# zhizdev/sparsefusion

Hardware: AMD Instinct MI355X
Metric: novel views/sec, distillation steps (2 NGP renders fwd+bwd + VAE enc/dec + 51-eval PLMS + LPIPS), 256^2 / 32x32 latents, 2-view synthetic hydrant (higher is better)
Workload: dtype bf16 MFMA operands / f32 accumulate (UNet); f32 (NGP render)

## Files before the change

### sparsefusion_amd/csrc/ngp_bwd_mfma.h

```cpp
#pragma once
#include "sf_dev.h"
#include "ngp_device.h"

#define FB_PTS 32
#define FB_SF 33
#define FB_SH 65
#define FB_WAVE_FLOATS (FB_PTS * FB_SF + 2 * FB_PTS * FB_SH + FB_PTS * 4 + FB_PTS)
#define FB_W0 0
#define FB_W1 (FB_W0 + NGP_HID * FB_SF)
#define FB_W2 (FB_W1 + NGP_HID * FB_SH)
#define FB_B0 (FB_W2 + NGP_OUT * NGP_HID)
#define FB_B1 (FB_B0 + NGP_HID)
#define FB_B2 (FB_B1 + NGP_HID)
#define FB_WTOT (FB_B2 + 8)
#define FB_LDS_FLOATS (FB_WTOT + 4 * FB_WAVE_FLOATS)

struct FBArgs {
  const float* table; const float* w0; const float* b0; const float* w1; const float* b1; const float* w2; const float* b2;
  float bound;
  long long* g_w0; long long* g_b0; long long* g_w1; long long* g_b1; long long* g_w2; long long* g_b2;
  float* f_w0; float* f_b0; float* f_w1; float* f_b1; float* f_w2; float* f_b2;
  float thr;
  NgpLevels lv;
  const float* rays_o; const float* rays_d; const float* aabb; const float* z_s; const float* dsig; const float* drgb;
  float* dfeat_out;
  uint32_t P, T2;
  uint32_t dfeat_P, p_off;
  const float* feat_c; const float* feat_f; const uint32_t* perm;
};

SF_KERNEL(256) void k_ngp_field_bwd_mfma(FBArgs a) {
  SF_DYN_LDS(lds_raw);
  float* W = reinterpret_cast<float*>(lds_raw);
  const int tid = threadIdx.x, lane = tid & 63, wave = tid >> 6;
  float* F = W + FB_WTOT + wave * FB_WAVE_FLOATS;
  float* H1 = F + FB_PTS * FB_SF;
  float* H2 = H1 + FB_PTS * FB_SH;
  float* DO = H2 + FB_PTS * FB_SH;
  float* INS = DO + FB_PTS * 4;
  for (int i = tid; i < NGP_HID * NGP_FEAT; i += 256) W[FB_W0 + (i >> 5) * FB_SF + (i & 31)] = a.w0[i];
  for (int i = tid; i < NGP_HID * NGP_HID; i += 256) W[FB_W1 + (i >> 6) * FB_SH + (i & 63)] = a.w1[i];
  for (int i = tid; i < NGP_OUT * NGP_HID; i += 256) W[FB_W2 + i] = a.w2[i];
  if (tid < NGP_HID) { W[FB_B0 + tid] = a.b0[tid]; W[FB_B1 + tid] = a.b1[tid]; }
  if (tid < NGP_OUT) W[FB_B2 + tid] = a.b2[tid];
  float box[6];
#pragma unroll
  for (int i = 0; i < 6; ++i) box[i] = a.aabb[i];
  sf_sync();

  const int li = lane & 15, kq = lane >> 4;
  f32x4 acc1[4][4], acc0[4][2];
#pragma unroll
  for (int i = 0; i < 4; ++i) {
#pragma unroll
    for (int j = 0; j < 4; ++j) acc1[i][j] = f32x4{0.f, 0.f, 0.f, 0.f};
    acc0[i][0] = f32x4{0.f, 0.f, 0.f, 0.f};
    acc0[i][1] = f32x4{0.f, 0.f, 0.f, 0.f};
  }
  float acc2[4] = {0.f, 0.f, 0.f, 0.f};
  float accb2 = 0.0f, accb1 = 0.0f, accb0 = 0.0f;

  const uint32_t n_trips = (a.P + FB_PTS - 1) / FB_PTS;
  for (uint32_t trip = blockIdx.x * 4 + wave; trip < n_trips; trip += gridDim.x * 4) {
    const uint32_t p0 = trip * FB_PTS;
    const int pl = lane & 31, half = lane >> 5;
    const uint32_t p = p0 + pl;
    const bool live = p < a.P;
    float x[3] = {0.f, 0.f, 0.f}, x01[3] = {0.f, 0.f, 0.f};
    bool inside = false;
    if (live) {
      const uint32_t n = p / a.T2;
      const float o[3] = {a.rays_o[n * 3], a.rays_o[n * 3 + 1], a.rays_o[n * 3 + 2]};
      const float d[3] = {a.rays_d[n * 3], a.rays_d[n * 3 + 1], a.rays_d[n * 3 + 2]};
      ngp_point(o, d, a.z_s[p], box, x);
      inside = ngp_unit(x, a.bound, x01);
    }
    if (a.feat_c) {
      f32x4 fv[4];
#pragma unroll
      for (int j = 0; j < 4; ++j) fv[j] = f32x4{0.f, 0.f, 0.f, 0.f};
      if (live) {
        const uint32_t pg = a.p_off + p, n = pg / a.T2, T = a.T2 >> 1;
        const uint32_t src = a.perm[pg];
        const float* row = (src < T ? a.feat_c + ((size_t)n * T + src) * NGP_FEAT : a.feat_f + ((size_t)n * T + (src - T)) * NGP_FEAT) + half * 16;
#pragma unroll
        for (int j = 0; j < 4; ++j) fv[j] = *reinterpret_cast<const f32x4*>(row + 4 * j);
      }
#pragma unroll
      for (int j = 0; j < 4; ++j)
#pragma unroll
        for (int e = 0; e < 4; ++e) F[pl * FB_SF + half * 16 + 4 * j + e] = fv[j][e];
    } else {
#pragma unroll
      for (int ll = 0; ll < 8; ++ll) {
        const uint32_t l = half * 8 + ll;
        float r0 = 0.0f, r1 = 0.0f;
        if (inside && l < a.lv.L) {
          NgpCell c;
          ngp_cell(a.lv, l, x01, c);
          const float* tab = a.table + (size_t)a.lv.offset[l] * 2;
#pragma unroll
          for (int i = 0; i < 8; ++i) {
            const f32x2 fv = *reinterpret_cast<const f32x2*>(tab + (size_t)c.row[i] * 2);
            r0 = fmaf(c.w[i], fv[0], r0);
            r1 = fmaf(c.w[i], fv[1], r1);
          }
        }
        F[pl * FB_SF + 2 * l] = r0;
        F[pl * FB_SF + 2 * l + 1] = r1;
      }
    }
    if (half == 0) INS[pl] = inside ? 1.0f : 0.0f;
    sf_wave_sync();

    {
      f32x4 c[2][4];
#pragma unroll
      for (int nt = 0; nt < 4; ++nt) {
        const float bv = W[FB_B0 + nt * 16 + li];
        c[0][nt] = f32x4{bv, bv, bv, bv};
        c[1][nt] = c[0][nt];
      }
#pragma unroll
      for (int s = 0; s < NGP_FEAT / 4; ++s) {
        const float a0 = F[li * FB_SF + 4 * s + kq], a1 = F[(16 + li) * FB_SF + 4 * s + kq];
#pragma unroll
        for (int nt = 0; nt < 4; ++nt) {
          const float b = W[FB_W0 + (nt * 16 + li) * FB_SF + 4 * s + kq];
          c[0][nt] = sf_mfma4(a0, b, c[0][nt]);
          c[1][nt] = sf_mfma4(a1, b, c[1][nt]);
        }
      }
#pragma unroll
      for (int mt = 0; mt < 2; ++mt)
#pragma unroll
        for (int nt = 0; nt < 4; ++nt)
#pragma unroll
          for (int r = 0; r < 4; ++r) H1[(mt * 16 + 4 * kq + r) * FB_SH + nt * 16 + li] = fmaxf(c[mt][nt][r], 0.0f);
    }
    sf_wave_sync();
    {
      f32x4 c[2][4];
#pragma unroll
      for (int nt = 0; nt < 4; ++nt) {
        const float bv = W[FB_B1 + nt * 16 + li];
        c[0][nt] = f32x4{bv, bv, bv, bv};
        c[1][nt] = c[0][nt];
      }
#pragma unroll
      for (int s = 0; s < NGP_HID / 4; ++s) {
        const float a0 = H1[li * FB_SH + 4 * s + kq], a1 = H1[(16 + li) * FB_SH + 4 * s + kq];
#pragma unroll
        for (int nt = 0; nt < 4; ++nt) {
          const float b = W[FB_W1 + (nt * 16 + li) * FB_SH + 4 * s + kq];
          c[0][nt] = sf_mfma4(a0, b, c[0][nt]);
          c[1][nt] = sf_mfma4(a1, b, c[1][nt]);
        }
      }
#pragma unroll
      for (int mt = 0; mt < 2; ++mt)
#pragma unroll
        for (int nt = 0; nt < 4; ++nt)
#pragma unroll
          for (int r = 0; r < 4; ++r) H2[(mt * 16 + 4 * kq + r) * FB_SH + nt * 16 + li] = fmaxf(c[mt][nt][r], 0.0f);
    }
    sf_wave_sync();
    {
      float o0 = W[FB_B2 + 2 * half], o1 = W[FB_B2 + 2 * half + 1];
#pragma unroll 8
      for (int k = 0; k < NGP_HID; ++k) {
        const float hk = H2[pl * FB_SH + k];
        o0 = fmaf(W[FB_W2 + (2 * half) * NGP_HID + k], hk, o0);
        o1 = fmaf(W[FB_W2 + (2 * half + 1) * NGP_HID + k], hk, o1);
      }
      float d0 = 0.0f, d1 = 0.0f;
      if (live) {
        if (half == 0) {
          const float pre = o0 + ngp_blob(x);
          d0 = a.dsig[p] * expf(fminf(fmaxf(pre, -15.0f), 15.0f));
          const float sg = ngp_sigmoid(o1);
          d1 = a.drgb[p * 3 + 0] * sg * (1.0f - sg);
        } else {
          const float s0 = ngp_sigmoid(o0), s1 = ngp_sigmoid(o1);
          d0 = a.drgb[p * 3 + 1] * s0 * (1.0f - s0);
          d1 = a.drgb[p * 3 + 2] * s1 * (1.0f - s1);
        }
      }
      DO[pl * 4 + 2 * half] = d0;
      DO[pl * 4 + 2 * half + 1] = d1;
    }
    sf_wave_sync();
    {
      float b = 0.0f;
#pragma unroll 4
      for (int q = 0; q < FB_PTS; ++q) {
        const float dv = DO[q * 4 + kq];
#pragma unroll
        for (int i = 0; i < 4; ++i) acc2[i] = fmaf(dv, H2[q * FB_SH + 4 * li + i], acc2[i]);
        b += dv;
      }
      if (li == 0) accb2 += b;
    }
    sf_wave_sync();
    {
      const float w0 = W[FB_W2 + lane], w1 = W[FB_W2 + NGP_HID + lane], w2 = W[FB_W2 + 2 * NGP_HID + lane],
                  w3 = W[FB_W2 + 3 * NGP_HID + lane];
      float b = 0.0f;
#pragma unroll 4
      for (int q = 0; q < FB_PTS; ++q) {
        const f32x4 dv = *reinterpret_cast<const f32x4*>(DO + q * 4);
        const float g = fmaf(w3, dv[3], fmaf(w2, dv[2], fmaf(w1, dv[1], w0 * dv[0])));
        const float m = H2[q * FB_SH + lane] > 0.0f ? g : 0.0f;
        H2[q * FB_SH + lane] = m;
        b += m;
      }
      accb1 += b;
    }
    sf_wave_sync();
#pragma unroll
    for (int s = 0; s < FB_PTS / 4; ++s) {
      float av[4], bv[4];
#pragma unroll
      for (int t = 0; t < 4; ++t) {
        av[t] = H2[(4 * s + kq) * FB_SH + t * 16 + li];
        bv[t] = H1[(4 * s + kq) * FB_SH + t * 16 + li];
      }
#pragma unroll
      for (int jt = 0; jt < 4; ++jt)
#pragma unroll
        for (int kt = 0; kt < 4; ++kt) acc1[jt][kt] = sf_mfma4(av[jt], bv[kt], acc1[jt][kt]);
    }
    {
      f32x4 c[2][4];
#pragma unroll
      for (int nt = 0; nt < 4; ++nt) { c[0][nt] = f32x4{0.f, 0.f, 0.f, 0.f}; c[1][nt] = c[0][nt]; }
#pragma unroll
      for (int s = 0; s < NGP_HID / 4; ++s) {
        const float a0 = H2[li * FB_SH + 4 * s + kq], a1 = H2[(16 + li) * FB_SH + 4 * s + kq];
#pragma unroll
        for (int nt = 0; nt < 4; ++nt) {
          const float b = W[FB_W1 + (4 * s + kq) * FB_SH + nt * 16 + li];
          c[0][nt] = sf_mfma4(a0, b, c[0][nt]);
          c[1][nt] = sf_mfma4(a1, b, c[1][nt]);
        }
      }
      sf_wave_sync();
#pragma unroll
      for (int mt = 0; mt < 2; ++mt)
#pragma unroll
        for (int nt = 0; nt < 4; ++nt)
#pragma unroll
          for (int r = 0; r < 4; ++r) {
            float* hp = H1 + (mt * 16 + 4 * kq + r) * FB_SH + nt * 16 + li;
            *hp = *hp > 0.0f ? c[mt][nt][r] : 0.0f;
          }
    }
    sf_wave_sync();
    {
      float b = 0.0f;
#pragma unroll 8
      for (int q = 0; q < FB_PTS; ++q) b += H1[q * FB_SH + lane];
      accb0 += b;
    }
#pragma unroll
    for (int s = 0; s < FB_PTS / 4; ++s) {
      float av[4], bv[2];
#pragma unroll
      for (int t = 0; t < 4; ++t) av[t] = H1[(4 * s + kq) * FB_SH + t * 16 + li];
      bv[0] = F[(4 * s + kq) * FB_SF + li];
      bv[1] = F[(4 * s + kq) * FB_SF + 16 + li];
#pragma unroll
      for (int jt = 0; jt < 4; ++jt) {
        acc0[jt][0] = sf_mfma4(av[jt], bv[0], acc0[jt][0]);
        acc0[jt][1] = sf_mfma4(av[jt], bv[1], acc0[jt][1]);
      }
    }
    if (a.dfeat_out) {
      f32x4 c[2][2];
      c[0][0] = c[0][1] = c[1][0] = c[1][1] = f32x4{0.f, 0.f, 0.f, 0.f};
#pragma unroll
      for (int s = 0; s < NGP_HID / 4; ++s) {
        const float a0 = H1[li * FB_SH + 4 * s + kq], a1 = H1[(16 + li) * FB_SH + 4 * s + kq];
        const float b0 = W[FB_W0 + (4 * s + kq) * FB_SF + li], b1 = W[FB_W0 + (4 * s + kq) * FB_SF + 16 + li];
        c[0][0] = sf_mfma4(a0, b0, c[0][0]);
        c[0][1] = sf_mfma4(a0, b1, c[0][1]);
        c[1][0] = sf_mfma4(a1, b0, c[1][0]);
        c[1][1] = sf_mfma4(a1, b1, c[1][1]);
      }
      sf_wave_sync();
#pragma unroll
      for (int mt = 0; mt < 2; ++mt)
#pragma unroll
        for (int ft = 0; ft < 2; ++ft)
#pragma unroll
          for (int r = 0; r < 4; ++r) {
            const int q = mt * 16 + 4 * kq + r, f = ft * 16 + li;
            F[q * FB_SF + f] = INS[q] != 0.0f ? c[mt][ft][r] : 0.0f;
          }
      sf_wave_sync();
      {
        const uint32_t l = lane >> 2, q0 = (lane & 3) * 8;
        if (l < a.lv.L) {
          float* dst = a.dfeat_out + ((size_t)l * a.dfeat_P + a.p_off + p0 + q0) * 2;
          if (p0 + FB_PTS <= a.P && !((a.dfeat_P | a.p_off) & 1)) {
#pragma unroll
            for (int j = 0; j < 4; ++j) {
              f32x4 v;
              v[0] = F[(q0 + 2 * j) * FB_SF + 2 * l];     v[1] = F[(q0 + 2 * j) * FB_SF + 2 * l + 1];
              v[2] = F[(q0 + 2 * j + 1) * FB_SF + 2 * l]; v[3] = F[(q0 + 2 * j + 1) * FB_SF + 2 * l + 1];
              *reinterpret_cast<f32x4*>(dst + 4 * j) = v;
            }
          } else {
            for (int j = 0; j < 8; ++j)
              if (p0 + q0 + j < a.P) { dst[2 * j] = F[(q0 + j) * FB_SF + 2 * l]; dst[2 * j + 1] = F[(q0 + j) * FB_SF + 2 * l + 1]; }
          }
        }
      }
    }
    sf_wave_sync();
  }

#pragma unroll
  for (int jt = 0; jt < 4; ++jt)
#pragma unroll
    for (int r = 0; r < 4; ++r) {
      const int j = jt * 16 + 4 * kq + r;
#pragma unroll
      for (int kt = 0; kt < 4; ++kt) sf_grad_add(a.g_w1 + j * NGP_HID + kt * 16 + li, a.f_w1 + j * NGP_HID + kt * 16 + li, acc1[jt][kt][r], a.thr);
      sf_grad_add(a.g_w0 + j * NGP_FEAT + li, a.f_w0 + j * NGP_FEAT + li, acc0[jt][0][r], a.thr);
      sf_grad_add(a.g_w0 + j * NGP_FEAT + 16 + li, a.f_w0 + j * NGP_FEAT + 16 + li, acc0[jt][1][r], a.thr);
    }
#pragma unroll
  for (int i = 0; i < 4; ++i) sf_grad_add(a.g_w2 + kq * NGP_HID + 4 * li + i, a.f_w2 + kq * NGP_HID + 4 * li + i, acc2[i], a.thr);
  if (li == 0) sf_grad_add(a.g_b2 + kq, a.f_b2 + kq, accb2, a.thr);
  sf_grad_add(a.g_b1 + lane, a.f_b1 + lane, accb1, a.thr);
  sf_grad_add(a.g_b0 + lane, a.f_b0 + lane, accb0, a.thr);
}
```

Baseline: 18.16.

## Prefetch next-trip inputs and move NGP backward output layer onto MFMA

Restructures the NGP field backward kernel into a templated per-wave routine that software-prefetches the next trip's ray, depth, upstream-gradient scalars and cached feature rows (with a two-ahead perm index) so global loads overlap the current trip's MLP work. The output layer forward and its weight gradient move from scalar FMA loops onto 4x4 MFMA ops, with W2 weights held in registers. Hidden activations are kept in registers for ReLU masking instead of being reread from LDS. This raises register pressure and could lower occupancy or cause spills.

```diff
diff --git a/sparsefusion_amd/csrc/ngp_bwd_mfma.h b/sparsefusion_amd/csrc/ngp_bwd_mfma.h
--- a/sparsefusion_amd/csrc/ngp_bwd_mfma.h
+++ b/sparsefusion_amd/csrc/ngp_bwd_mfma.h
@@ -29,67 +29,117 @@
   const float* feat_c; const float* feat_f; const uint32_t* perm;
 };
 
-SF_KERNEL(256) void k_ngp_field_bwd_mfma(FBArgs a) {
-  SF_DYN_LDS(lds_raw);
-  float* W = reinterpret_cast<float*>(lds_raw);
+struct FBPre { float z, g0, g1, o[3], d[3]; };
+
+SF_DEV void fb_fetch_scalars(const FBArgs& a, uint32_t trip, uint32_t n_trips, int pl, int half, FBPre& q) {
+  q.z = q.g0 = q.g1 = 0.0f;
+#pragma unroll
+  for (int i = 0; i < 3; ++i) q.o[i] = q.d[i] = 0.0f;
+  if (trip < n_trips) {
+    const uint32_t p = trip * FB_PTS + pl;
+    if (p < a.P) {
+      const uint32_t n = p / a.T2;
+#pragma unroll
+      for (int i = 0; i < 3; ++i) { q.o[i] = a.rays_o[n * 3 + i]; q.d[i] = a.rays_d[n * 3 + i]; }
+      q.z = a.z_s[p];
+      q.g0 = half ? a.drgb[p * 3 + 1] : a.dsig[p];
+      q.g1 = half ? a.drgb[p * 3 + 2] : a.drgb[p * 3 + 0];
+    }
+  }
+}
+SF_DEV uint32_t fb_fetch_perm(const FBArgs& a, uint32_t trip, uint32_t n_trips, int pl) {
+  uint32_t src = 0;
+  if (trip < n_trips) {
+    const uint32_t p = trip * FB_PTS + pl;
+    if (p < a.P) src = a.perm[a.p_off + p];
+  }
+  return src;
+}
+SF_DEV void fb_fetch_row(const FBArgs& a, uint32_t trip, uint32_t n_trips, int pl, int half, uint32_t src, f32x4 fv[4]) {
+#pragma unroll
+  for (int j = 0; j < 4; ++j) fv[j] = f32x4{0.f, 0.f, 0.f, 0.f};
+  if (trip < n_trips) {
+    const uint32_t p = trip * FB_PTS + pl;
+    if (p < a.P) {
+      const uint32_t pg = a.p_off + p, n = pg / a.T2, T = a.T2 >> 1;
+      const float* row = (src < T ? a.feat_c + ((size_t)n * T + src) * NGP_FEAT : a.feat_f + ((size_t)n * T + (src - T)) * NGP_FEAT) + half * 16;
+#pragma unroll
+      for (int j = 0; j < 4; ++j) fv[j] = *reinterpret_cast<const f32x4*>(row + 4 * j);
+    }
+  }
+}
+template <bool CACHE>
+SF_DEV void fb_wave(const FBArgs& a, float* W, const float box[6]) {
   const int tid = threadIdx.x, lane = tid & 63, wave = tid >> 6;
   float* F = W + FB_WTOT + wave * FB_WAVE_FLOATS;
   float* H1 = F + FB_PTS * FB_SF;
   float* H2 = H1 + FB_PTS * FB_SH;
   float* DO = H2 + FB_PTS * FB_SH;
   float* INS = DO + FB_PTS * 4;
-  for (int i = tid; i < NGP_HID * NGP_FEAT; i += 256) W[FB_W0 + (i >> 5) * FB_SF + (i & 31)] = a.w0[i];
-  for (int i = tid; i < NGP_HID * NGP_HID; i += 256) W[FB_W1 + (i >> 6) * FB_SH + (i & 63)] = a.w1[i];
-  for (int i = tid; i < NGP_OUT * NGP_HID; i += 256) W[FB_W2 + i] = a.w2[i];
-  if (tid < NGP_HID) { W[FB_B0 + tid] = a.b0[tid]; W[FB_B1 + tid] = a.b1[tid]; }
-  if (tid < NGP_OUT) W[FB_B2 + tid] = a.b2[tid];
-  float box[6];
-#pragma unroll
-  for (int i = 0; i < 6; ++i) box[i] = a.aabb[i];
-  sf_sync();
-
   const int li = lane & 15, kq = lane >> 4;
-  f32x4 acc1[4][4], acc0[4][2];
+  const int pl = lane & 31, half = lane >> 5;
+  const bool out_lane = li < NGP_OUT;
+  float w2b[NGP_HID / 4], w2c[NGP_OUT][4];
+#pragma unroll
+  for (int s = 0; s < NGP_HID / 4; ++s) {
+    const float v = W[FB_W2 + (li & 3) * NGP_HID + 4 * s + kq];
+    w2b[s] = out_lane ? v : 0.0f;
+  }
+#pragma unroll
+  for (int o = 0; o < NGP_OUT; ++o)
+#pragma unroll
+    for (int nt = 0; nt < 4; ++nt) w2c[o][nt] = W[FB_W2 + o * NGP_HID + nt * 16 + li];
+  const float b2v = out_lane ? W[FB_B2 + (li & 3)] : 0.0f;
+
+  f32x4 acc1[4][4], acc0[4][2], acc2[4];
 #pragma unroll
   for (int i = 0; i < 4; ++i) {
 #pragma unroll
     for (int j = 0; j < 4; ++j) acc1[i][j] = f32x4{0.f, 0.f, 0.f, 0.f};
     acc0[i][0] = f32x4{0.f, 0.f, 0.f, 0.f};
     acc0[i][1] = f32x4{0.f, 0.f, 0.f, 0.f};
-  }
-  float acc2[4] = {0.f, 0.f, 0.f, 0.f};
+    acc2[i] = f32x4{0.f, 0.f, 0.f, 0.f};
+  }
   float accb2 = 0.0f, accb1 = 0.0f, accb0 = 0.0f;
 
   const uint32_t n_trips = (a.P + FB_PTS - 1) / FB_PTS;
+  const uint32_t trip_step = gridDim.x * 4;
+  FBPre nx;
+  f32x4 nx_fv[4];
+  uint32_t nx_src = 0;
+  {
+    const uint32_t trip0 = blockIdx.x * 4 + wave;
+    fb_fetch_scalars(a, trip0, n_trips, pl, half, nx);
+    if (CACHE) {
+      const uint32_t src0 = fb_fetch_perm(a, trip0, n_trips, pl);
+      nx_src = fb_fetch_perm(a, trip0 + trip_step, n_trips, pl);
+      fb_fetch_row(a, trip0, n_trips, pl, half, src0, nx_fv);
+    } else {
+#pragma unroll
+      for (int j = 0; j < 4; ++j) nx_fv[j] = f32x4{0.f, 0.f, 0.f, 0.f};
+    }
+  }
   for (uint32_t trip = blockIdx.x * 4 + wave; trip < n_trips; trip += gridDim.x * 4) {
     const uint32_t p0 = trip * FB_PTS;
-    const int pl = lane & 31, half = lane >> 5;
     const uint32_t p = p0 + pl;
     const bool live = p < a.P;
+    const FBPre cur = nx;
     float x[3] = {0.f, 0.f, 0.f}, x01[3] = {0.f, 0.f, 0.f};
     bool inside = false;
     if (live) {
-      const uint32_t n = p / a.T2;
-      const float o[3] = {a.rays_o[n * 3], a.rays_o[n * 3 + 1], a.rays_o[n * 3 + 2]};
-      const float d[3] = {a.rays_d[n * 3], a.rays_d[n * 3 + 1], a.rays_d[n * 3 + 2]};
-      ngp_point(o, d, a.z_s[p], box, x);
+      ngp_point(cur.o, cur.d, cur.z, box, x);
       inside = ngp_unit(x, a.bound, x01);
     }
-    if (a.feat_c) {
-      f32x4 fv[4];
-#pragma unroll
-      for (int j = 0; j < 4; ++j) fv[j] = f32x4{0.f, 0.f, 0.f, 0.f};
-      if (live) {
-        const uint32_t pg = a.p_off + p, n = pg / a.T2, T = a.T2 >> 1;
-        const uint32_t src = a.perm[pg];
-        const float* row = (src < T ? a.feat_c + ((size_t)n * T + src) * NGP_FEAT : a.feat_f + ((size_t)n * T + (src - T)) * NGP_FEAT) + half * 16;
-#pragma unroll
-        for (int j = 0; j < 4; ++j) fv[j] = *reinterpret_cast<const f32x4*>(row + 4 * j);
-      }
+    if (CACHE) {
 #pragma unroll
       for (int j = 0; j < 4; ++j)
 #pragma unroll
-        for (int e = 0; e < 4; ++e) F[pl * FB_SF + half * 16 + 4 * j + e] = fv[j][e];
+        for (int e = 0; e < 4; ++e) F[pl * FB_SF + half * 16 + 4 * j + e] = nx_fv[j][e];
+    }
+    fb_fetch_scalars(a, trip + trip_step, n_trips, pl, half, nx);
+    if (CACHE) {
+      fb_fetch_row(a, trip + trip_step, n_trips, pl, half, nx_src, nx_fv);
+      nx_src = fb_fetch_perm(a, trip + 2 * trip_step, n_trips, pl);
     } else {
 #pragma unroll
       for (int ll = 0; ll < 8; ++ll) {
@@ -113,13 +163,14 @@
     if (half == 0) INS[pl] = inside ? 1.0f : 0.0f;
     sf_wave_sync();
 
-    {
-      f32x4 c[2][4];
+    f32x4 h1[2][4];
+    {
 #pragma unroll
       for (int nt = 0; nt < 4; ++nt) {
         const float bv = W[FB_B0 + nt * 16 + li];
-        c[0][nt] = f32x4{bv, bv, bv, bv};
-        c[1][nt] = c[0][nt];
+        h1[0][nt] = f32x4{bv, bv, bv, bv};
+        h1[1][nt] = h1[0][nt];
+        SF_USE_FROM_HERE(h1[1][nt]);
       }
 #pragma unroll
       for (int s = 0; s < NGP_FEAT / 4; ++s) {
@@ -127,8 +178,8 @@
 #pragma unroll
         for (int nt = 0; nt < 4; ++nt) {
           const float b = W[FB_W0 + (nt * 16 + li) * FB_SF + 4 * s + kq];
-          c[0][nt] = sf_mfma4(a0, b, c[0][nt]);
-          c[1][nt] = sf_mfma4(a1, b, c[1][nt]);
+          h1[0][nt] = sf_mfma4(a0, b, h1[0][nt]);
+          h1[1][nt] = sf_mfma4(a1, b, h1[1][nt]);
         }
       }
 #pragma unroll
@@ -136,16 +187,20 @@
 #pragma unroll
         for (int nt = 0; nt < 4; ++nt)
 #pragma unroll
-          for (int r = 0; r < 4; ++r) H1[(mt * 16 + 4 * kq + r) * FB_SH + nt * 16 + li] = fmaxf(c[mt][nt][r], 0.0f);
-    }
-    sf_wave_sync();
-    {
-      f32x4 c[2][4];
+          for (int r = 0; r < 4; ++r) {
+            h1[mt][nt][r] = fmaxf(h1[mt][nt][r], 0.0f);
+            H1[(mt * 16 + 4 * kq + r) * FB_SH + nt * 16 + li] = h1[mt][nt][r];
+          }
+    }
+    sf_wave_sync();
+    f32x4 h2[2][4];
+    {
 #pragma unroll
       for (int nt = 0; nt < 4; ++nt) {
         const float bv = W[FB_B1 + nt * 16 + li];
-        c[0][nt] = f32x4{bv, bv, bv, bv};
-        c[1][nt] = c[0][nt];
+        h2[0][nt] = f32x4{bv, bv, bv, bv};
+        h2[1][nt] = h2[0][nt];
+        SF_USE_FROM_HERE(h2[1][nt]);
       }
 #pragma unroll
       for (int s = 0; s < NGP_HID / 4; ++s) {
@@ -153,8 +208,8 @@
 #pragma unroll
         for (int nt = 0; nt < 4; ++nt) {
           const float b = W[FB_W1 + (nt * 16 + li) * FB_SH + 4 * s + kq];
-          c[0][nt] = sf_mfma4(a0, b, c[0][nt]);
-          c[1][nt] = sf_mfma4(a1, b, c[1][nt]);
+          h2[0][nt] = sf_mfma4(a0, b, h2[0][nt]);
+          h2[1][nt] = sf_mfma4(a1, b, h2[1][nt]);
         }
       }
 #pragma unroll
@@ -162,28 +217,43 @@
 #pragma unroll
         for (int nt = 0; nt < 4; ++nt)
 #pragma unroll
-          for (int r = 0; r < 4; ++r) H2[(mt * 16 + 4 * kq + r) * FB_SH + nt * 16 + li] = fmaxf(c[mt][nt][r], 0.0f);
-    }
-    sf_wave_sync();
-    {
-      float o0 = W[FB_B2 + 2 * half], o1 = W[FB_B2 + 2 * half + 1];
-#pragma unroll 8
-      for (int k = 0; k < NGP_HID; ++k) {
-        const float hk = H2[pl * FB_SH + k];
-        o0 = fmaf(W[FB_W2 + (2 * half) * NGP_HID + k], hk, o0);
-        o1 = fmaf(W[FB_W2 + (2 * half + 1) * NGP_HID + k], hk, o1);
-      }
+          for (int r = 0; r < 4; ++r) {
+            h2[mt][nt][r] = fmaxf(h2[mt][nt][r], 0.0f);
+            H2[(mt * 16 + 4 * kq + r) * FB_SH + nt * 16 + li] = h2[mt][nt][r];
+          }
+    }
+    sf_wave_sync();
+    {
+      f32x4 co[2];
+      co[0] = f32x4{b2v, b2v, b2v, b2v};
+      co[1] = co[0];
+      SF_USE_FROM_HERE(co[1]);
+#pragma unroll
+      for (int s = 0; s < NGP_HID / 4; ++s) {
+        const float a0 = H2[li * FB_SH + 4 * s + kq], a1 = H2[(16 + li) * FB_SH + 4 * s + kq];
+        co[0] = sf_mfma4(a0, w2b[s], co[0]);
+        co[1] = sf_mfma4(a1, w2b[s], co[1]);
+      }
+      if (out_lane) {
+#pragma unroll
+        for (int mt = 0; mt < 2; ++mt)
+#pragma unroll
+          for (int r = 0; r < 4; ++r) DO[(mt * 16 + 4 * kq + r) * 4 + li] = co[mt][r];
+      }
+      sf_wave_sync();
+      const f32x2 ov = *reinterpret_cast<const f32x2*>(DO + pl * 4 + 2 * half);
+      const float o0 = ov[0], o1 = ov[1];
       float d0 = 0.0f, d1 = 0.0f;
       if (live) {
         if (half == 0) {
           const float pre = o0 + ngp_blob(x);
-          d0 = a.dsig[p] * expf(fminf(fmaxf(pre, -15.0f), 15.0f));
+          d0 = cur.g0 * expf(fminf(fmaxf(pre, -15.0f), 15.0f));
           const float sg = ngp_sigmoid(o1);
-          d1 = a.drgb[p * 3 + 0] * sg * (1.0f - sg);
+          d1 = cur.g1 * sg * (1.0f - sg);
         } else {
           const float s0 = ngp_sigmoid(o0), s1 = ngp_sigmoid(o1);
-          d0 = a.drgb[p * 3 + 1] * s0 * (1.0f - s0);
-          d1 = a.drgb[p * 3 + 2] * s1 * (1.0f - s1);
+          d0 = cur.g0 * s0 * (1.0f - s0);
+          d1 = cur.g1 * s1 * (1.0f - s1);
         }
       }
       DO[pl * 4 + 2 * half] = d0;
@@ -191,32 +261,46 @@
     }
     sf_wave_sync();
     {
+#pragma unroll
+      for (int s = 0; s < FB_PTS / 4; ++s) {
+        const float v = DO[(4 * s + kq) * 4 + (li & 3)];
+        const float av = out_lane ? v : 0.0f;
+#pragma unroll
+        for (int nt = 0; nt < 4; ++nt) acc2[nt] = sf_mfma4(av, H2[(4 * s + kq) * FB_SH + nt * 16 + li], acc2[nt]);
+      }
       float b = 0.0f;
-#pragma unroll 4
-      for (int q = 0; q < FB_PTS; ++q) {
-        const float dv = DO[q * 4 + kq];
-#pragma unroll
-        for (int i = 0; i < 4; ++i) acc2[i] = fmaf(dv, H2[q * FB_SH + 4 * li + i], acc2[i]);
-        b += dv;
-      }
+#pragma unroll 8
+      for (int q = 0; q < FB_PTS; ++q) b += DO[q * 4 + kq];
       if (li == 0) accb2 += b;
     }
-    sf_wave_sync();
-    {
-      const float w0 = W[FB_W2 + lane], w1 = W[FB_W2 + NGP_HID + lane], w2 = W[FB_W2 + 2 * NGP_HID + lane],
-                  w3 = W[FB_W2 + 3 * NGP_HID + lane];
+    {
+      f32x4 g[2][4];
+#pragma unroll
+      for (int mt = 0; mt < 2; ++mt)
+#pragma unroll
+        for (int r = 0; r < 4; ++r) {
+          const f32x4 dv = *reinterpret_cast<const f32x4*>(DO + (mt * 16 + 4 * kq + r) * 4);
+#pragma unroll
+          for (int nt = 0; nt < 4; ++nt) {
+            const float v = fmaf(w2c[3][nt], dv[3], fmaf(w2c[2][nt], dv[2], fmaf(w2c[1][nt], dv[1], w2c[0][nt] * dv[0])));
+            g[mt][nt][r] = h2[mt][nt][r] > 0.0f ? v : 0.0f;
+          }
+        }
+      sf_wave_sync();
+#pragma unroll
+      for (int mt = 0; mt < 2; ++mt)
+#pragma unroll
+        for (int nt = 0; nt < 4; ++nt)
+#pragma unroll
+          for (int r = 0; r < 4; ++r) H2[(mt * 16 + 4 * kq + r) * FB_SH + nt * 16 + li] = g[mt][nt][r];
+    }
+    sf_wave_sync();
+    {
       float b = 0.0f;
-#pragma unroll 4
-      for (int q = 0; q < FB_PTS; ++q) {
-        const f32x4 dv = *reinterpret_cast<const f32x4*>(DO + q * 4);
-        const float g = fmaf(w3, dv[3], fmaf(w2, dv[2], fmaf(w1, dv[1], w0 * dv[0])));
-        const float m = H2[q * FB_SH + lane] > 0.0f ? g : 0.0f;
-        H2[q * FB_SH + lane] = m;
-        b += m;
-      }
+#pragma unroll 8
+      for (int q = 0; q < FB_PTS; ++q) b += H2[q * FB_SH + lane];
       accb1 += b;
     }
-    sf_wave_sync();
 #pragma unroll
     for (int s = 0; s < FB_PTS / 4; ++s) {
       float av[4], bv[4];
@@ -250,10 +334,8 @@
 #pragma unroll
         for (int nt = 0; nt < 4; ++nt)
 #pragma unroll
-          for (int r = 0; r < 4; ++r) {
-            float* hp = H1 + (mt * 16 + 4 * kq + r) * FB_SH + nt * 16 + li;
-            *hp = *hp > 0.0f ? c[mt][nt][r] : 0.0f;
-          }
+          for (int r = 0; r < 4; ++r)
+            H1[(mt * 16 + 4 * kq + r) * FB_SH + nt * 16 + li] = h1[mt][nt][r] > 0.0f ? c[mt][nt][r] : 0.0f;
     }
     sf_wave_sync();
     {
@@ -330,9 +412,30 @@
       sf_grad_add(a.g_w0 + j * NGP_FEAT + li, a.f_w0 + j * NGP_FEAT + li, acc0[jt][0][r], a.thr);
       sf_grad_add(a.g_w0 + j * NGP_FEAT + 16 + li, a.f_w0 + j * NGP_FEAT + 16 + li, acc0[jt][1][r], a.thr);
     }
-#pragma unroll
-  for (int i = 0; i < 4; ++i) sf_grad_add(a.g_w2 + kq * NGP_HID + 4 * li + i, a.f_w2 + kq * NGP_HID + 4 * li + i, acc2[i], a.thr);
+  if (kq == 0) {
+#pragma unroll
+    for (int nt = 0; nt < 4; ++nt)
+#pragma unroll
+      for (int r = 0; r < 4; ++r) sf_grad_add(a.g_w2 + r * NGP_HID + nt * 16 + li, a.f_w2 + r * NGP_HID + nt * 16 + li, acc2[nt][r], a.thr);
+  }
   if (li == 0) sf_grad_add(a.g_b2 + kq, a.f_b2 + kq, accb2, a.thr);
   sf_grad_add(a.g_b1 + lane, a.f_b1 + lane, accb1, a.thr);
   sf_grad_add(a.g_b0 + lane, a.f_b0 + lane, accb0, a.thr);
 }
+
+SF_KERNEL(256) void k_ngp_field_bwd_mfma(FBArgs a) {
+  SF_DYN_LDS(lds_raw);
+  float* W = reinterpret_cast<float*>(lds_raw);
+  const int tid = threadIdx.x;
+  for (int i = tid; i < NGP_HID * NGP_FEAT; i += 256) W[FB_W0 + (i >> 5) * FB_SF + (i & 31)] = a.w0[i];
+  for (int i = tid; i < NGP_HID * NGP_HID; i += 256) W[FB_W1 + (i >> 6) * FB_SH + (i & 63)] = a.w1[i];
+  for (int i = tid; i < NGP_OUT * NGP_HID; i += 256) W[FB_W2 + i] = a.w2[i];
+  if (tid < NGP_HID) { W[FB_B0 + tid] = a.b0[tid]; W[FB_B1 + tid] = a.b1[tid]; }
+  if (tid < NGP_OUT) W[FB_B2 + tid] = a.b2[tid];
+  float box[6];
+#pragma unroll
+  for (int i = 0; i < 6; ++i) box[i] = a.aabb[i];
+  sf_sync();
+  if (a.feat_c) fb_wave<true>(a, W, box);
+  else fb_wave<false>(a, W, box);
+}
```

Measured after the change: 18.29 (median of 6 runs). Within noise of the previous version (+0.7%).
